# PotatoSpudowski/fastLLaMa

Measured on NVIDIA H100. Metric: tokens/sec LLaMA-7B q4_0 decode (n_batch=1, greedy), higher is better.
Workload: dtype u8

## Files before the change

fastllama_b200/csrc/fl_token_kernel.cu:

```cuda
#include <cuda_fp16.h>
#include <stdlib.h>

#include <algorithm>
#include <vector>

#include "fl_common.cuh"
#include "fl_decode.h"
#include "fl_decode_dev.cuh"
#include "fl_exact.cuh"
#include "fl_kernels.h"

#define TK_CW 16
#define TK_NT (TK_CW * 32)
#define TK_TG 4
#define TK_WPG 4
#define TK_GMAX 4
#define TK_CHB 32
#define TK_PW 4
#define TK_THREADS (TK_NT + 32 * TK_PW)
#define TK_REGS_CONSUMER 104
#define TK_REGS_PRODUCER 64

enum { TK_PH_MATVEC = 0, TK_PH_ATTN = 1 };

struct tk_phase {
    int kind;
    int nb, nchunks;
    uint32_t srow;
    int swiglu;
    int units[3];
    uint32_t row_bytes;
    fl_mv_args a;
    const float *q, *kcache, *vcache;
    float *out;
    int k_row_stride, n_head, head_dim, n_ctx;
    int head_split;
    int out_ll, out_seq, n_out_peer;
    float *out_peer[7];
    float scale;
};

struct tk_params {
    const tk_phase *phases;
    int n_phases;
    unsigned *grid_bar;
    unsigned *err;
    int rank, world;
    unsigned *ll_count;
    int n_ll;
    const uint16_t *exp_tab;
    unsigned long long *prof;
    unsigned *prof2;
    int S, Sg;
    uint32_t grid_magic, grid_shift, s_magic, s_shift;
    uint32_t slot_bytes;
    int diag;
    uint32_t off_y, off_red, off_rowbuf, off_cnt, off_sc, off_stage0;
};

__device__ __forceinline__ unsigned long long tk_now() {
    unsigned long long t;
    asm volatile("mov.u64 %0, %globaltimer;" : "=l"(t));
    return t;
}
__device__ __forceinline__ void tk_bar_consumers(int id) { asm volatile("bar.sync %0, %1;" ::"r"(id), "r"(TK_NT) : "memory"); }

__device__ __forceinline__ void tk_wait_ge(const unsigned *p, unsigned target, bool sys, unsigned *err, unsigned who) {
    unsigned long long t0 = 0;
    for (unsigned n = 1;; n++) {
        unsigned v;
        if (sys) asm volatile("ld.relaxed.sys.global.u32 %0, [%1];" : "=r"(v) : "l"(p) : "memory");
        else asm volatile("ld.acquire.gpu.global.u32 %0, [%1];" : "=r"(v) : "l"(p) : "memory");
        if ((int)(v - target) >= 0) return;
        if ((n & 1023u) == 0) {
            if (*(volatile unsigned *)err) return;
            const unsigned long long t = tk_now();
            if (t0 == 0) t0 = t;
            else if (t - t0 > 2000000000ull) {
                if (atomicExch(err, 1u) == 0u) { err[1] = who; err[2] = target; err[3] = v; err[4] = blockIdx.x; }
                return;
            }
        }
    }
}
__device__ __forceinline__ void tk_mbar_wait(uint32_t bar, uint32_t parity, unsigned *err, unsigned who, unsigned slot) {
    unsigned long long t0 = 0;
    for (unsigned n = 1; !fl_mbar_try_wait(bar, parity); n++) {
        if ((n & 4095u) == 0) {
            if (*(volatile unsigned *)err) return;
            const unsigned long long t = tk_now();
            if (t0 == 0) t0 = t;
            else if (t - t0 > 2000000000ull) {
                if (atomicExch(err, 1u) == 0u) { err[1] = who; err[2] = slot; err[3] = parity; err[4] = blockIdx.x; }
                return;
            }
        }
    }
}
__device__ __forceinline__ void tk_tag_wait(volatile uint32_t *tag, uint32_t want, unsigned *err, unsigned who, unsigned slot) {
    unsigned long long t0 = 0;
    for (unsigned n = 1; *tag != want; n++) {
        if ((n & 4095u) == 0) {
            if (*(volatile unsigned *)err) return;
            const unsigned long long t = tk_now();
            if (t0 == 0) t0 = t;
            else if (t - t0 > 2000000000ull) {
                if (atomicExch(err, 1u) == 0u) { err[1] = who; err[2] = slot; err[3] = want; err[4] = blockIdx.x; }
                return;
            }
        }
    }
}
__device__ __forceinline__ void tk_grid_sync(const tk_params &prm, unsigned target, unsigned) {
    tk_bar_consumers(13);
    if (threadIdx.x == 0) {
        asm volatile("red.release.gpu.global.add.u32 [%0], 1;" ::"l"(prm.grid_bar) : "memory");
        tk_wait_ge(prm.grid_bar, target, false, prm.err, 0x100u);
    }
    tk_bar_consumers(13);
}

struct tk_slice {
    int f0, f1, f2, n0, n1, n2, t0, t1, ntiles;
};
__device__ __forceinline__ uint32_t tk_div(uint32_t n, uint32_t magic, uint32_t shift) { return (magic ? __umulhi(n, magic) : n) >> shift; }
__device__ __forceinline__ tk_slice tk_make_slice_u(int m0, int m1, int m2, int lgG, uint32_t grid_magic, uint32_t grid_shift) {
    tk_slice sl;
    const unsigned U = (unsigned)(m0 + m1 + m2);
    const int u0 = (int)tk_div(U * blockIdx.x, grid_magic, grid_shift);
    const int u1 = (int)tk_div(U * (blockIdx.x + 1), grid_magic, grid_shift);
    const int rnd = (1 << lgG) - 1;
    fd_seg_span(u0, u1, 0, m0, sl.f0, sl.n0);
    fd_seg_span(u0, u1, m0, m1, sl.f1, sl.n1);
    fd_seg_span(u0, u1, m0 + m1, m2, sl.f2, sl.n2);
    sl.t0 = (sl.n0 + rnd) >> lgG;
    sl.t1 = sl.t0 + ((sl.n1 + rnd) >> lgG);
    sl.ntiles = sl.t1 + ((sl.n2 + rnd) >> lgG);
    return sl;
}
__device__ __forceinline__ void tk_tile_of(const tk_slice &sl, int G, int t, int &seg, int &unit0, int &nunits) {
    seg = (t < sl.t0) ? 0 : (t < sl.t1) ? 1 : 2;
    const int j = t - (seg == 0 ? 0 : seg == 1 ? sl.t0 : sl.t1);
    const int first = seg == 0 ? sl.f0 : seg == 1 ? sl.f1 : sl.f2;
    const int n = seg == 0 ? sl.n0 : seg == 1 ? sl.n1 : sl.n2;
    unit0 = first + j * G;
    nunits = min(G, n - j * G);
}

typedef fl_yx tk_yblock;

template <int E>
__device__ __forceinline__ void tk_load_vals(const float4 *p4, int u, float v[E], bool cg) {
#pragma unroll
    for (int k = 0; k < E / 4; k++) {
        const float4 t = cg ? __ldcg(p4 + (E / 4) * u + k) : __ldg(p4 + (E / 4) * u + k);
        v[4 * k + 0] = t.x; v[4 * k + 1] = t.y; v[4 * k + 2] = t.z; v[4 * k + 3] = t.w;
    }
}
template <int E>
__device__ __forceinline__ void tk_zero_vals(float v[E]) {
#pragma unroll
    for (int k = 0; k < E; k++) v[k] = 0.f;
}
template <int E>
__device__ __forceinline__ void tk_load_ll(const float *base, int u, float v[E], unsigned e, unsigned *err) {
    const uint4 *p = (const uint4 *)base + (size_t)(E / 2) * u;
    unsigned long long t0 = 0;
    for (unsigned n = 1;; n++) {
        uint4 t[E / 2];
#pragma unroll
        for (int k = 0; k < E / 2; k++)
            asm volatile("ld.relaxed.sys.global.v4.u32 {%0, %1, %2, %3}, [%4];" : "=r"(t[k].x), "=r"(t[k].y), "=r"(t[k].z), "=r"(t[k].w) : "l"(p + k) : "memory");
        bool ok = true;
#pragma unroll
        for (int k = 0; k < E / 2; k++) {
            ok = ok && t[k].y == e && t[k].w == e;
            v[2 * k] = __uint_as_float(t[k].x);
            v[2 * k + 1] = __uint_as_float(t[k].z);
        }
        if (ok) return;
        __nanosleep(n < 4 ? 40u : 200u);
        if ((n & 255u) == 0) {
            if (*(volatile unsigned *)err) return;
            const unsigned long long now = tk_now();
            if (t0 == 0) t0 = now;
            else if (now - t0 > 2000000000ull) {
                if (atomicExch(err, 1u) == 0u) { err[1] = 0x300u; err[2] = e; err[3] = t[0].y; err[4] = blockIdx.x; }
                return;
            }
        }
    }
}
template <int E>
__device__ __forceinline__ void tk_load_x(const fl_mv_args &A, int u, float v[E], unsigned ll_epoch, unsigned *err) {
    if (A.x_ll) tk_load_ll<E>(A.x, u, v, ll_epoch, err);
    else tk_load_vals<E>((const float4 *)A.x, u, v, true);
    if (A.xadd) {
        float w[E];
        tk_load_vals<E>((const float4 *)A.xadd, u, w, true);
#pragma unroll
        for (int k = 0; k < E; k++) v[k] = __fadd_rn(v[k], w[k]);
    }
}
template <int E>
__device__ __forceinline__ void tk_store_vals(float *dst, int u, const float v[E]) {
#pragma unroll
    for (int k = 0; k < E / 4; k++) ((float4 *)dst)[(E / 4) * u + k] = make_float4(v[4 * k], v[4 * k + 1], v[4 * k + 2], v[4 * k + 3]);
}
template <int E>
__device__ __forceinline__ void tk_quant(const float v[E], int u, bool valid, tk_yblock *ysm, int off) {
    float m0 = 0.f, m1 = 0.f;
#pragma unroll
    for (int k = 0; k < E; k += 2) { m0 = fmaxf(m0, fabsf(v[k])); m1 = fmaxf(m1, fabsf(v[k + 1])); }
    float amax = fmaxf(m0, m1);
    if (E <= 16) amax = fmaxf(amax, __shfl_xor_sync(0xffffffffu, amax, 1));
    if (E == 8) amax = fmaxf(amax, __shfl_xor_sync(0xffffffffu, amax, 2));
    const float d = __fdiv_rn(amax, 127.f);
    const float id = (amax != 0.0f) ? __fdiv_rn(127.f, amax) : 0.0f;
    int q[E], s0 = 0, s1 = 0;
#pragma unroll
    for (int k = 0; k < E; k += 2) {
        q[k] = max(-128, min(127, __float2int_rn(__fmul_rn(v[k], id))));
        q[k + 1] = max(-128, min(127, __float2int_rn(__fmul_rn(v[k + 1], id))));
        s0 += q[k]; s1 += q[k + 1];
    }
    int sum = s0 + s1;
    if (E <= 16) sum += __shfl_xor_sync(0xffffffffu, sum, 1);
    if (E == 8) sum += __shfl_xor_sync(0xffffffffu, sum, 2);
    if (valid) {
        constexpr int NW = E / 8;
        constexpr int UPB = 32 / E;
        tk_yblock *yb = ysm + u / UPB;
        const int part = u % UPB;
#pragma unroll
        for (int j = 0; j < NW; j++) {
            const uint32_t ya = (uint32_t)(q[8 * j + 0] & 0xFF) | ((uint32_t)(q[8 * j + 1] & 0xFF) << 8) | ((uint32_t)(q[8 * j + 2] & 0xFF) << 16) | ((uint32_t)(q[8 * j + 3] & 0xFF) << 24);
            const uint32_t yb4 = (uint32_t)(q[8 * j + 4] & 0xFF) | ((uint32_t)(q[8 * j + 5] & 0xFF) << 8) | ((uint32_t)(q[8 * j + 6] & 0xFF) << 16) | ((uint32_t)(q[8 * j + 7] & 0xFF) << 24);
            const int sa = q[8 * j + 0] + q[8 * j + 1] + q[8 * j + 2] + q[8 * j + 3], sb = q[8 * j + 4] + q[8 * j + 5] + q[8 * j + 6] + q[8 * j + 7];
            *(uint4 *)yb->q[NW * part + j] = make_uint4(ya, yb4, (uint32_t)(FX_MAGIC_I - off * sa), (uint32_t)(FX_MAGIC_I - off * sb));
        }
        if (part == 0) *(float2 *)&yb->d = make_float2(d, __fmul_rn(d, (float)sum));
    }
}
template <int E>
__device__ __forceinline__ void tk_prologue_nonorm(const fl_mv_args &A, int K, tk_yblock *ysm, int warp, int tid, unsigned lle, unsigned *err) {
    const int qoff = (A.type == FL_TYPE_Q4_0) ? 8 : 0;
    const int nu = K / E;
    if (E == 16 && A.pro != FL_PRO_SILUMUL && nu > TK_NT && nu <= 2 * TK_NT) {
        const int ua = tid, ub = tid + TK_NT;
        const bool vb = ub < nu, wb = TK_NT + warp * 32 < nu;
        float va[E], vv[E];
        tk_load_x<E>(A, ua, va, lle, err);
        if (vb) tk_load_x<E>(A, ub, vv, lle, err); else tk_zero_vals<E>(vv);
        if (A.sum_out && blockIdx.x == 0) { tk_store_vals<E>(A.sum_out, ua, va); if (vb) tk_store_vals<E>(A.sum_out, ub, vv); }
        tk_quant<E>(va, ua, true, ysm, qoff);
        if (wb) tk_quant<E>(vv, ub, vb, ysm, qoff);
        return;
    }
    for (int u0 = 0; u0 < nu; u0 += TK_NT) {
        if (u0 + warp * 32 >= nu) break;
        const int u = u0 + tid;
        const bool valid = u < nu;
        float v[E];
        if (valid) tk_load_x<E>(A, u, v, lle, err); else tk_zero_vals<E>(v);
        if (A.sum_out && blockIdx.x == 0 && valid) tk_store_vals<E>(A.sum_out, u, v);
        if (A.pro == FL_PRO_SILUMUL) {
            float bm[E];
            if (valid) tk_load_vals<E>((const float4 *)A.b, u, bm, true); else tk_zero_vals<E>(bm);
#pragma unroll
            for (int k = 0; k < E; k++) {
                const uint16_t hh = __half_as_ushort(__float2half_rn(v[k]));
                v[k] = __fmul_rn(__half2float(__ushort_as_half(__ldg(A.silu_tab + hh))), bm[k]);
            }
        }
        tk_quant<E>(v, u, valid, ysm, qoff);
    }
}

template <int RES>
__device__ __forceinline__ void tk_prologue_norm(const fl_mv_args &A, int K, tk_yblock *ysm, double *red, int warp, int lane, int tid, unsigned lle, unsigned *err) {
    const int qoff = (A.type == FL_TYPE_Q4_0) ? 8 : 0;
    constexpr int E = 8, NR = RES > 0 ? RES : 1;
    const int nu = K >> 3;
    float v[NR][E], gm[NR][E];
    double acc = 0.0;
    if (RES > 0) {
#pragma unroll
        for (int r = 0; r < NR; r++) {
            const int u = tid + r * TK_NT;
            if (u < nu) { tk_load_x<E>(A, u, v[r], lle, err); tk_load_vals<E>((const float4 *)A.gamma, u, gm[r], false); }
            else { tk_zero_vals<E>(v[r]); tk_zero_vals<E>(gm[r]); }
        }
#pragma unroll
        for (int r = 0; r < NR; r++)
#pragma unroll
            for (int k = 0; k < E; k++) acc += (double)__fmul_rn(v[r][k], v[r][k]);
    } else {
        for (int u = tid; u < nu; u += TK_NT) {
            tk_load_x<E>(A, u, v[0], lle, err);
#pragma unroll
            for (int k = 0; k < E; k++) acc += (double)__fmul_rn(v[0][k], v[0][k]);
        }
    }
    acc = fl_warp_sum_d(acc);
    if (lane == 0) red[warp] = acc;
    tk_bar_consumers(15);
    if (warp == 0) {
        double t = 0.0;
#pragma unroll
        for (int w = 0; w < TK_CW; w++) t += red[w];
        const float mean = (float)(t / (double)K);
        if (lane == 0) ((float *)(red + 16))[0] = __fdiv_rn(1.0f, __fsqrt_rn(__fadd_rn(mean, 1e-6f)));
    }
    tk_bar_consumers(15);
    const float scale = ((float *)(red + 16))[0];
    if (RES > 0) {
#pragma unroll
        for (int r = 0; r < NR; r++) {
            if (r * TK_NT + warp * 32 < nu) {
                const int u = tid + r * TK_NT;
                const bool valid = u < nu;
                if (A.sum_out && blockIdx.x == 0 && valid) tk_store_vals<E>(A.sum_out, u, v[r]);
#pragma unroll
                for (int k = 0; k < E; k++) v[r][k] = __fmul_rn(gm[r][k], __fmul_rn(v[r][k], scale));
                if (A.normed_out && blockIdx.x == 0 && valid) tk_store_vals<E>(A.normed_out, u, v[r]);
                tk_quant<E>(v[r], u, valid, ysm, qoff);
            }
        }
    } else {
        for (int u0 = 0; u0 < nu; u0 += TK_NT) {
            if (u0 + warp * 32 >= nu) break;
            const int u = u0 + tid;
            const bool valid = u < nu;
            if (valid) { tk_load_x<E>(A, u, v[0], lle, err); tk_load_vals<E>((const float4 *)A.gamma, u, gm[0], false); }
            else { tk_zero_vals<E>(v[0]); tk_zero_vals<E>(gm[0]); }
            if (A.sum_out && blockIdx.x == 0 && valid) tk_store_vals<E>(A.sum_out, u, v[0]);
#pragma unroll
            for (int k = 0; k < E; k++) v[0][k] = __fmul_rn(gm[0][k], __fmul_rn(v[0][k], scale));
            if (A.normed_out && blockIdx.x == 0 && valid) tk_store_vals<E>(A.normed_out, u, v[0]);
            tk_quant<E>(v[0], u, valid, ysm, qoff);
        }
    }
}

__device__ __forceinline__ void tk_prologue(const fl_mv_args &A, int K, tk_yblock *ysm, double *red, int warp, int lane, int tid, unsigned lle, unsigned *err) {
    const int nu8 = K >> 3;
    if (A.pro == FL_PRO_RMSNORM) {
        if (nu8 <= TK_NT) tk_prologue_norm<1>(A, K, ysm, red, warp, lane, tid, lle, err);
        else if (nu8 <= 2 * TK_NT) tk_prologue_norm<2>(A, K, ysm, red, warp, lane, tid, lle, err);
        else tk_prologue_norm<0>(A, K, ysm, red, warp, lane, tid, lle, err);
    } else if (nu8 <= TK_NT) {
        tk_prologue_nonorm<8>(A, K, ysm, warp, tid, lle, err);
    } else {
        tk_prologue_nonorm<16>(A, K, ysm, warp, tid, lle, err);
    }
}

__device__ __forceinline__ void tk_store_ll(float *slot, int row, float v, unsigned e, float *const *peers, int n_peers) {
    const unsigned uv = __float_as_uint(v);
    asm volatile("st.relaxed.sys.global.v2.u32 [%0], {%1, %2};" ::"l"(slot + 2 * row), "r"(uv), "r"(e) : "memory");
    for (int r = 0; r < n_peers; r++)
        asm volatile("st.relaxed.sys.global.v2.u32 [%0], {%1, %2};" ::"l"(peers[r] + 2 * row), "r"(uv), "r"(e) : "memory");
}
__device__ __forceinline__ float2 tk_epilogue_preload(const tk_phase &ph, int seg, int u, int n_past) {
    const fl_mv_args &A = ph.a;
    if (ph.swiglu) return make_float2(0.f, 0.f);
    const int r2 = 2 * u;
    if (A.epi == FL_EPI_QKV) {
        if (seg < 2) return __ldg((const float2 *)A.rope_cs + (size_t)n_past * (A.head_dim >> 1) + ((r2 % A.head_dim) >> 1));
        return make_float2(0.f, 0.f);
    }
    if (A.epi == FL_EPI_RESADD) {
        if (A.res_ll) {
            const float4 t = __ldcg((const float4 *)(A.res + 2 * r2));
            return make_float2(t.x, t.z);
        }
        return __ldcg((const float2 *)(A.res + r2));
    }
    return make_float2(0.f, 0.f);
}
__device__ __forceinline__ void tk_epilogue(const tk_phase &ph, int seg, int u, float a, float b, int n_past, float2 pre, unsigned ll_epoch) {
    const fl_mv_args &A = ph.a;
    if (ph.swiglu) {
        const uint16_t h = __half_as_ushort(__float2half_rn(a));
        const float o = __fmul_rn(__half2float(__ushort_as_half(__ldg(A.silu_tab + h))), b);
        if (A.out_ll) tk_store_ll(A.seg_dst[0], u, o, ll_epoch, A.dst_peer, A.n_dst_peer);
        else A.seg_dst[0][u] = o;
        return;
    }
    const int r2 = 2 * u;
    if (A.epi == FL_EPI_QKV) {
        if (seg < 2) {
            const float2 cs = pre;
            const float y0 = __fmaf_rn(a, cs.x, -__fmul_rn(b, cs.y));
            const float y1 = __fmaf_rn(a, cs.y, __fmul_rn(b, cs.x));
            float *o = (seg == 0) ? (A.seg_dst[0] + r2) : (A.kcache + (size_t)n_past * A.n_embd + r2);
            *(float2 *)o = make_float2(y0, y1);
        } else {
            A.vcache[(size_t)r2 * A.n_ctx + n_past] = a;
            A.vcache[(size_t)(r2 + 1) * A.n_ctx + n_past] = b;
        }
        return;
    }
    if (A.epi == FL_EPI_RESADD) {
        a = __fadd_rn(a, pre.x);
        b = __fadd_rn(b, pre.y);
    }
    if (A.out_ll) {
        tk_store_ll(A.seg_dst[seg], r2, a, ll_epoch, A.dst_peer, A.n_dst_peer);
        tk_store_ll(A.seg_dst[seg], r2 + 1, b, ll_epoch, A.dst_peer, A.n_dst_peer);
        return;
    }
    *(float2 *)(A.seg_dst[seg] + r2) = make_float2(a, b);
}

struct tk_stream {
    int first, n_g;
};
__device__ __forceinline__ tk_stream tk_stream_of(int g, int T0, int ntasks) {
    tk_stream st;
    st.first = ((g - (T0 & 3)) + 4) & 3;
    st.n_g = st.first < ntasks ? (ntasks - st.first + 3) >> 2 : 0;
    return st;
}
__device__ __forceinline__ void tk_slot_of(const tk_params &prm, int g, uint32_t idx, int &s, uint32_t &par) {
    const uint32_t q = tk_div(idx, prm.s_magic, prm.s_shift);
    s = (int)(idx - q * (uint32_t)prm.Sg) * TK_TG + g;
    par = q & 1u;
}

__device__ __forceinline__ unsigned tk_clock() {
    unsigned c;
    asm volatile("mov.u32 %0, %%clock;" : "=r"(c));
    return c;
}
template <int TYPE, bool PROF>
__device__ __forceinline__ void tk_consume(const tk_phase &ph, const tk_params &prm, const tk_slice &sl, int T0, uint32_t &cg, const tk_yblock *ysm,
                                           uint8_t *stage0, volatile uint32_t *tags, uint32_t bar0, int warp, int lane, unsigned *pw, unsigned lle) {
    unsigned c_begin = 0, c_wait = 0, c_dot = 0, c_tail = 0, c_rounds = 0, c_t = 0;
    if (PROF) { c_begin = tk_clock(); c_t = c_begin; }
    constexpr int BB = (TYPE == FL_TYPE_Q4_0) ? 20 : 24, QOFF = (TYPE == FL_TYPE_Q4_0) ? 4 : 8;
    const fl_mv_args &A = ph.a;
    const int S = prm.S;
    const int g = warp % TK_TG, wl = warp / TK_TG;
    const int r = lane >> 2, jj = lane & 3;
    const bool swiglu = ph.swiglu != 0;
    const int C = ph.nchunks, nb = ph.nb;
    const tk_stream st = tk_stream_of(g, T0, sl.ntiles);
    const int n_past = (A.epi == FL_EPI_QKV) ? *A.n_past : 0;
    const bool leader = swiglu ? ((lane & 3) == 0 && lane < 16) : ((lane & 7) == 0);
    const int pr = swiglu ? (lane >> 2) : (lane >> 3);
    const uint32_t row_off = (uint32_t)r * ph.srow + (uint32_t)(QOFF + 4 * jj);
    for (int k = wl; k < st.n_g; k += TK_WPG) {
        const int k0 = k - wl, n_r = min(TK_WPG, st.n_g - k0);
        int seg, unit0, nunits;
        tk_tile_of(sl, TK_GMAX, st.first + 4 * k, seg, unit0, nunits);
        float2 pre = make_float2(0.f, 0.f);
        if (leader && pr < nunits) pre = tk_epilogue_preload(ph, seg, unit0 + pr, n_past);
        float a0 = 0.0f, a1 = 0.0f, sm = 0.0f;
        for (int c = 0; c < C; c++) {
            int s;
            uint32_t par;
            const uint32_t idx = cg + (uint32_t)(k0 * C + c * n_r + wl);
            tk_slot_of(prm, g, idx, s, par);
            tk_tag_wait(tags + s, idx + 1u, prm.err, 0x600u + (unsigned)warp, (unsigned)s);
            tk_mbar_wait(bar0 + 8u * s, par, prm.err, 0x400u + (unsigned)warp, (unsigned)s);
            if (PROF) { const unsigned t = tk_clock(); c_wait += t - c_t; c_t = t; c_rounds++; }
            if (!(prm.diag & 2)) {
                const uint8_t *wp = stage0 + (size_t)s * prm.slot_bytes + row_off;
                const tk_yblock *yp = ysm + c * TK_CHB;
                const int nbc = min(TK_CHB, nb - c * TK_CHB);
#pragma unroll 8
                for (int i = 0; i < nbc; i++) {
                    const uint32_t w = *(const uint32_t *)(wp + i * BB);
                    const float dx = *(const float *)(wp + i * BB - (QOFF + 4 * jj));
                    const uint4 y = *(const uint4 *)yp[i].q[jj];
                    const float2 ds = *(const float2 *)&yp[i].d;
                    if (TYPE == FL_TYPE_Q4_1) sm = __fmaf_rn(*(const float *)(wp + i * BB - (QOFF + 4 * jj) + 4), ds.y, sm);
                    fx_block(w, __fmul_rn(dx, ds.x), y, a0, a1);
                }
            }
            __syncwarp();
            if (lane == 0) fl_mbar_arrive(bar0 + 8u * (S + s));
            if (PROF) { const unsigned t = tk_clock(); c_dot += t - c_t; c_t = t; }
        }
        float tot = fx_reduce(a0, a1);
        if (TYPE == FL_TYPE_Q4_1) tot = __fadd_rn(tot, sm);
        const float other = __shfl_down_sync(0xffffffffu, tot, swiglu ? 16 : 4);
        if (leader && pr < nunits) tk_epilogue(ph, seg, unit0 + pr, tot, other, n_past, pre, lle);
        if (PROF) { const unsigned t = tk_clock(); c_tail += t - c_t; c_t = t; }
    }
    cg += (uint32_t)(st.n_g * C);
    if (PROF && lane == 0 && pw) {
        pw[0] = 0; pw[1] = c_wait; pw[2] = c_dot; pw[3] = c_tail; pw[4] = c_rounds; pw[5] = tk_clock() - c_begin; pw[6] = (unsigned)sl.ntiles; pw[7] = 0;
    }
}

__device__ __forceinline__ void tk_attention(const tk_phase &ph, const tk_params &prm, float *sc, double *red, int head, int part_id, int warp, int lane, int tid, unsigned lle_out) {
    float *redf = (float *)(red + 20);
    const int hd = ph.head_dim;
    const int n_pos = *ph.a.n_past + 1;
    const float *q = ph.q + (size_t)head * hd;
    const float *kbase = ph.kcache + (size_t)head * hd;
    if (hd == 128) {
        float qe[4];
#pragma unroll
        for (int c = 0; c < 4; c++) qe[c] = __ldcg(q + lane + 32 * c);
        for (int j0 = warp * 8; j0 < n_pos; j0 += TK_CW * 8) {
            float kv[8][4], acc[8];
#pragma unroll
            for (int u = 0; u < 8; u++)
#pragma unroll
                for (int c = 0; c < 4; c++) kv[u][c] = __ldcg(kbase + (size_t)min(j0 + u, n_pos - 1) * ph.k_row_stride + lane + 32 * c);
#pragma unroll
            for (int u = 0; u < 8; u++) {
                acc[u] = 0.f;
#pragma unroll
                for (int c = 0; c < 4; c++) acc[u] = __fmaf_rn(kv[u][c], qe[c], acc[u]);
            }
#pragma unroll
            for (int u = 0; u < 8; u++) {
                const float a = fx_reduce_f32(acc[u]);
                if (lane == 0 && j0 + u < n_pos) sc[j0 + u] = __fmul_rn(a, ph.scale);
            }
        }
    } else {
        for (int j0 = warp * 4; j0 < n_pos; j0 += TK_CW * 4) {
            float acc[4] = {0.f, 0.f, 0.f, 0.f};
            for (int e = lane; e < hd; e += 32) {
                const float qe = __ldcg(q + e);
#pragma unroll
                for (int u = 0; u < 4; u++) acc[u] = __fmaf_rn(__ldcg(kbase + (size_t)min(j0 + u, n_pos - 1) * ph.k_row_stride + e), qe, acc[u]);
            }
#pragma unroll
            for (int u = 0; u < 4; u++) {
                const float a = fx_reduce_f32(acc[u]);
                if (lane == 0 && j0 + u < n_pos) sc[j0 + u] = __fmul_rn(a, ph.scale);
            }
        }
    }
    tk_bar_consumers(12);
    float mx = -INFINITY;
    for (int j = tid; j < n_pos; j += TK_NT) mx = fmaxf(mx, sc[j]);
    mx = fl_warp_max(mx);
    if (lane == 0) redf[warp] = mx;
    tk_bar_consumers(12);
    mx = redf[0];
    for (int w = 1; w < TK_CW; w++) mx = fmaxf(mx, redf[w]);
    double sum = 0.0;
    for (int j = tid; j < n_pos; j += TK_NT) {
        const uint16_t hh = __half_as_ushort(__float2half_rn(__fsub_rn(sc[j], mx)));
        const float e = __half2float(__ushort_as_half(__ldg(prm.exp_tab + hh)));
        sc[j] = e;
        sum += (double)e;
    }
    sum = fl_warp_sum_d(sum);
    if (lane == 0) red[warp] = sum;
    tk_bar_consumers(12);
    double tot = 0.0;
    for (int w = 0; w < TK_CW; w++) tot += red[w];
    const float inv = (float)(1.0 / tot);
    for (int j = tid; j < n_pos; j += TK_NT) sc[j] = __fmul_rn(sc[j], inv);
    tk_bar_consumers(12);
    const int dpc = hd / ph.head_split;
    const int np = n_pos & ~31, rem = n_pos - np, nma = fx_left_nma(rem);
    for (int dl = warp; dl < dpc; dl += TK_CW) {
        const int d = part_id * dpc + dl;
        const float *vrow = ph.vcache + ((size_t)head * hd + d) * ph.n_ctx;
        float acc = 0.0f;
        const float lx = (lane < rem) ? __ldcg(vrow + np + lane) : 0.0f, ly = (lane < rem) ? sc[np + lane] : 0.0f;
        const float lv = __fmul_rn(lx, ly);
        for (int k = lane; k < np; k += 32) acc = __fmaf_rn(__ldcg(vrow + k), sc[k], acc);
        float o = fx_reduce_f32(acc);
        for (int k = 0; k < nma; k++) o = __fadd_rn(o, __shfl_sync(0xffffffffu, lv, k));
        for (int k = nma; k < rem; k++) o = __fmaf_rn(__shfl_sync(0xffffffffu, lx, k), __shfl_sync(0xffffffffu, ly, k), o);
        if (lane == 0) {
            if (ph.out_ll) tk_store_ll(ph.out, head * hd + d, o, lle_out, ph.out_peer, ph.n_out_peer);
            else ph.out[(size_t)head * hd + d] = o;
        }
    }
}
__device__ __forceinline__ void tk_attention_prefetch(const tk_phase &ph, int head, int part_id, int tid) {
    const int hd = ph.head_dim, n_past = *ph.a.n_past;
    const int kl = (hd * 4 + 127) / 128;
    for (int i = tid; i < n_past * kl; i += TK_NT) {
        const float *p = ph.kcache + (size_t)(i / kl) * ph.k_row_stride + (size_t)head * hd + (i % kl) * 32;
        asm volatile("prefetch.global.L2 [%0];" ::"l"(p));
    }
    const int dpc = hd / ph.head_split;
    const int vl = (n_past * 4 + 127) / 128;
    for (int i = tid; i < dpc * vl; i += TK_NT) {
        const float *p = ph.vcache + ((size_t)head * hd + part_id * dpc + i / vl) * ph.n_ctx + (i % vl) * 32;
        asm volatile("prefetch.global.L2 [%0];" ::"l"(p));
    }
}

template <bool PROF>
__global__ void __launch_bounds__(TK_THREADS, 1) k_decode_token(const tk_params prm) {
    extern __shared__ __align__(128) uint8_t smem[];
    uint64_t *bars = (uint64_t *)smem;
    volatile uint32_t *tags = (volatile uint32_t *)(smem + (size_t)16 * prm.S);
    tk_yblock *ysm = (tk_yblock *)(smem + prm.off_y);
    double *red = (double *)(smem + prm.off_red);
    float *sc = (float *)(smem + prm.off_sc);
    uint8_t *stage0 = smem + prm.off_stage0;
    __shared__ __align__(16) tk_phase phs[2];
    __shared__ tk_slice sl_sh;
    const int S = prm.S;
    const int warp = threadIdx.x >> 5, lane = threadIdx.x & 31;
    const uint32_t bar0 = fl_smem_u32(bars);

    if (warp >= TK_CW) {
        asm volatile("setmaxnreg.dec.sync.aligned.u32 %0;" ::"n"(TK_REGS_PRODUCER));
        const int pg = warp - TK_CW;
        if (pg == 0 && lane == 0) {
            for (int s = 0; s < S; s++) {
                fl_mbar_init(bar0 + 8u * s, 1);
                fl_mbar_init(bar0 + 8u * (S + s), 1);
                tags[s] = 0u;
            }
            fl_mbar_fence_init();
        }
        __syncwarp();
        asm volatile("bar.sync 14, %0;" ::"r"(TK_THREADS) : "memory");
        {
            const uint64_t pol = fl_policy_evict_first();
            int T0 = 0;
            uint32_t cg = 0;
            for (int pi = 0; pi < prm.n_phases; pi++) {
                const tk_phase *gp = prm.phases + pi;
                if (__ldg(&gp->kind) != TK_PH_MATVEC) continue;
                const int swiglu = __ldg(&gp->swiglu), C = __ldg(&gp->nchunks), nb = __ldg(&gp->nb), type = __ldg(&gp->a.type);
                const int m0 = __ldg(&gp->units[0]), m1 = __ldg(&gp->units[1]), m2 = __ldg(&gp->units[2]);
                const uint32_t row_bytes = __ldg(&gp->row_bytes), srow = __ldg(&gp->srow);
                const uint32_t bb = (type == FL_TYPE_Q4_0) ? 20u : 24u;
                const uint8_t *w0 = (const uint8_t *)__ldg((const unsigned long long *)&gp->a.seg_w[0]);
                const uint8_t *w1 = (const uint8_t *)__ldg((const unsigned long long *)&gp->a.seg_w[1]);
                const uint8_t *w2 = (const uint8_t *)__ldg((const unsigned long long *)&gp->a.seg_w[2]);
                const tk_slice sl = tk_make_slice_u(m0, m1, m2, 2, prm.grid_magic, prm.grid_shift);
                const tk_stream st = tk_stream_of(pg, T0, sl.ntiles);
                for (int k0 = 0; k0 < st.n_g; k0 += TK_WPG) {
                    const int n_r = min(TK_WPG, st.n_g - k0);
                    for (int c = 0; c < C; c++) {
                        const uint32_t cbytes = (uint32_t)min(TK_CHB, nb - c * TK_CHB) * bb;
                        for (int wl = 0; wl < n_r; wl++) {
                            int seg, unit0, nunits;
                            tk_tile_of(sl, TK_GMAX, st.first + 4 * (k0 + wl), seg, unit0, nunits);
                            int s;
                            uint32_t par;
                            const uint32_t idx = cg + (uint32_t)(k0 * C + c * n_r + wl);
                            tk_slot_of(prm, pg, idx, s, par);
                            const uint8_t *src = nullptr;
                            if (lane < 8) {
                                if (swiglu) { if ((lane & 3) < nunits) src = ((lane < 4) ? w0 : w1) + (size_t)(unit0 + (lane & 3)) * row_bytes; }
                                else if (lane < 2 * nunits) src = (seg == 0 ? w0 : seg == 1 ? w1 : w2) + (size_t)(2 * unit0 + lane) * row_bytes;
                            }
                            if (lane == 0) {
                                tk_mbar_wait(bar0 + 8u * (S + s), par ^ 1u, prm.err, 0x500u + (unsigned)pg, (unsigned)s);
                                tags[s] = idx + 1u;
                                if (prm.diag & 1) fl_mbar_arrive(bar0 + 8u * s);
                                else fl_mbar_expect_tx(bar0 + 8u * s, 2u * (uint32_t)nunits * cbytes);
                            }
                            __syncwarp();
                            if (src && !(prm.diag & 1))
                                fl_bulk_g2s_hint(fl_smem_u32(stage0 + (size_t)s * prm.slot_bytes + (size_t)lane * srow), src + (size_t)c * (TK_CHB * bb), cbytes, bar0 + 8u * s, pol);
                        }
                    }
                }
                cg += (uint32_t)(st.n_g * C);
                T0 += sl.ntiles;
            }
        }
        return;
    }

    asm volatile("setmaxnreg.inc.sync.aligned.u32 %0;" ::"n"(TK_REGS_CONSUMER));
    const int tid = threadIdx.x;
    static_assert(sizeof(tk_phase) % 4 == 0 && sizeof(tk_phase) / 4 <= TK_NT, "descriptor copy is one word per thread");
    if (warp == TK_CW - 1)
        for (int i = lane; i < (int)(sizeof(tk_phase) / 4); i += 32) ((uint32_t *)&phs[0])[i] = ((const uint32_t *)&prm.phases[0])[i];
    tk_bar_consumers(15);
    asm volatile("bar.sync 14, %0;" ::"r"(TK_THREADS) : "memory");
    int T0 = 0;
    uint32_t cg = 0;
    unsigned epoch = 0;
    unsigned ll_base = 0;
    if (prm.n_ll > 0) asm volatile("ld.relaxed.gpu.global.u32 %0, [%1];" : "=r"(ll_base) : "l"(prm.ll_count) : "memory");
    unsigned *err = prm.err;
    for (int pi = 0; pi < prm.n_phases; pi++) {
        const tk_phase &ph = phs[pi & 1];
        unsigned long long *pr = (prm.prof && tid == 0) ? prm.prof + ((size_t)pi * gridDim.x + blockIdx.x) * 4 : nullptr;
        if (pr) pr[0] = tk_now();
        const bool attn_here = ph.kind == TK_PH_ATTN && (int)blockIdx.x < ph.n_head * ph.head_split;
        const int a_head = attn_here ? (int)blockIdx.x / ph.head_split : 0, a_part = attn_here ? (int)blockIdx.x % ph.head_split : 0;
        if (attn_here) tk_attention_prefetch(ph, a_head, a_part, tid);
        const bool ll_in = ph.kind == TK_PH_MATVEC && ph.a.x_ll;
        const unsigned lle_in = ll_in ? ll_base + (unsigned)ph.a.x_seq + 1u : 0u;
        const unsigned lle_out = ph.kind == TK_PH_MATVEC ? (ph.a.out_ll ? ll_base + (unsigned)ph.a.out_seq + 1u : 0u) : (ph.out_ll ? ll_base + (unsigned)ph.out_seq + 1u : 0u);
        if (pi > 0 && ll_in) {
            tk_bar_consumers(13);
        } else if (pi > 0) {
            epoch++;
            if (!(prm.diag & 4)) tk_grid_sync(prm, epoch * gridDim.x, 0u);
            else tk_bar_consumers(13);
        }
        if (pr) pr[1] = tk_now();
        uint32_t next_word = 0;
        const bool copies = tid < (int)(sizeof(tk_phase) / 4) && pi + 1 < prm.n_phases;
        if (copies) next_word = __ldcg((const uint32_t *)&prm.phases[pi + 1] + tid);
        if (ph.kind == TK_PH_ATTN) {
            if (attn_here && !(prm.diag & 16)) tk_attention(ph, prm, sc, red, a_head, a_part, warp, lane, tid, lle_out);
            if (copies) ((uint32_t *)&phs[(pi + 1) & 1])[tid] = next_word;
            tk_bar_consumers(15);
            if (pr) pr[2] = pr[3] = tk_now();
            continue;
        }
        const int K = ph.nb * 32;
        if (tid == TK_NT - 1) sl_sh = tk_make_slice_u(ph.units[0], ph.units[1], ph.units[2], 2, prm.grid_magic, prm.grid_shift);
        if (!(prm.diag & 8)) tk_prologue(ph.a, K, ysm, red, warp, lane, tid, lle_in, err);
        if (copies) ((uint32_t *)&phs[(pi + 1) & 1])[tid] = next_word;
        tk_bar_consumers(15);
        if (pr) pr[2] = tk_now();
        const tk_slice &sl = sl_sh;
        unsigned *pw = (PROF && prm.prof2) ? prm.prof2 + (((size_t)pi * gridDim.x + blockIdx.x) * TK_CW + warp) * 8 : nullptr;
        if (ph.a.type == FL_TYPE_Q4_0) tk_consume<FL_TYPE_Q4_0, PROF>(ph, prm, sl, T0, cg, ysm, stage0, tags, bar0, warp, lane, pw, lle_out);
        else                           tk_consume<FL_TYPE_Q4_1, PROF>(ph, prm, sl, T0, cg, ysm, stage0, tags, bar0, warp, lane, pw, lle_out);
        T0 += sl.ntiles;
        if (pr) pr[3] = tk_now();
    }
    if (prm.n_ll > 0 && blockIdx.x == 0 && tid == 0) *prm.ll_count = ll_base + (unsigned)prm.n_ll;
}

struct fl_token_plan_impl {
    tk_phase *d_phases = nullptr;
    unsigned *d_bar = nullptr;
    unsigned *h_err = nullptr;
    unsigned long long *d_prof = nullptr;
    unsigned *d_prof2 = nullptr;
    tk_params prm;
    size_t smem = 0;
    int n_kernels = 0;
};

static void tk_magic(uint32_t d, uint32_t &magic, uint32_t &shift) {
    uint32_t k = 0;
    while ((2u << k) <= d) k++;
    shift = k;
    magic = ((d & (d - 1)) == 0) ? 0u : (uint32_t)((((uint64_t)1 << (32 + k)) + d - 1) / d);
}

static int tk_geometry(tk_phase &ph, size_t &tile_bytes) {
    const fl_mv_args &a = ph.a;
    const int bb = fl_block_bytes(a.type);
    const int nb = a.K / 32;
    const size_t row_bytes = a.row_stride_bytes ? a.row_stride_bytes : (size_t)nb * bb;
    FL_REQUIRE(bb > 0 && a.K > 0 && a.K % 32 == 0 && row_bytes % 16 == 0, "token kernel: unsupported matrix K=%d", a.K);
    const uint32_t chunk_bytes = (uint32_t)std::min(nb, TK_CHB) * bb;
    FL_REQUIRE(chunk_bytes % 16 == 0 && ((size_t)nb * bb) % 16 == 0, "token kernel: K=%d gives row pieces that are not multiples of 16 bytes", a.K);
    const uint32_t srow = (chunk_bytes / 16) % 2 ? chunk_bytes : chunk_bytes + 16;
    ph.units[0] = ph.units[1] = ph.units[2] = 0;
    if (ph.swiglu) {
        ph.units[0] = a.seg_rows[0];
    } else {
        for (int i = 0; i < a.nseg; i++) {
            FL_REQUIRE(a.seg_rows[i] > 0 && a.seg_rows[i] % 2 == 0, "token kernel: segment %d has an odd row count", i);
            ph.units[i] = a.seg_rows[i] / 2;
        }
    }
    for (int i = 0; i < a.nseg; i++) {
        FL_REQUIRE(((uintptr_t)a.seg_w[i] & 15) == 0, "token kernel: segment %d is not 16-byte aligned", i);
        FL_REQUIRE(a.epi == FL_EPI_QKV || ph.swiglu || ((uintptr_t)a.seg_dst[i] & 7) == 0, "token kernel: output %d is not 8-byte aligned", i);
    }
    FL_REQUIRE(a.epi != FL_EPI_RESADD || ((uintptr_t)a.res & 7) == 0, "token kernel: residual is not 8-byte aligned");
    FL_REQUIRE((long)ph.units[0] + ph.units[1] + ph.units[2] < (1 << 23), "token kernel: too many rows");
    ph.kind = TK_PH_MATVEC;
    ph.nb = nb; ph.nchunks = (nb + TK_CHB - 1) / TK_CHB; ph.srow = srow; ph.row_bytes = (uint32_t)row_bytes;
    tile_bytes = (size_t)2 * TK_GMAX * srow;
    return 0;
}

int flk_token_plan_create(const fl_token_step *steps, int n_steps, const uint16_t *silu_tab, const uint16_t *exp_tab, const void *rope_cs, unsigned *epoch_counter, void **out) {
    std::vector<tk_phase> phases((size_t)n_steps);
    for (int i = 0; i < n_steps; i++) {
        tk_phase &ph = phases[i];
        memset(&ph, 0, sizeof(ph));
        if (steps[i].kind == 1) {
            ph.kind = TK_PH_ATTN;
            ph.q = steps[i].q; ph.kcache = steps[i].kcache; ph.vcache = steps[i].vcache; ph.out = steps[i].out;
            ph.k_row_stride = steps[i].k_row_stride; ph.n_head = steps[i].n_head; ph.head_dim = steps[i].head_dim; ph.n_ctx = steps[i].n_ctx;
            ph.scale = steps[i].scale;
            ph.a.n_past = steps[i].n_past;
            ph.out_ll = steps[i].out_ll; ph.out_seq = steps[i].out_seq; ph.n_out_peer = steps[i].n_out_peer;
            for (int r = 0; r < 7; r++) ph.out_peer[r] = steps[i].out_peer[r];
        } else {
            ph.kind = TK_PH_MATVEC;
            ph.a = steps[i].mv;
            ph.a.silu_tab = silu_tab;
            ph.a.rope_cs = rope_cs;
        }
    }
    for (int i = 0; i < n_steps; i++)
        if (phases[i].kind == TK_PH_MATVEC && phases[i].a.swiglu) {
            const fl_mv_args &a = phases[i].a;
            FL_REQUIRE(a.nseg == 2 && a.epi == FL_EPI_STORE && a.seg_rows[0] == a.seg_rows[1], "token kernel: a swiglu step needs two equal segments and a plain store");
            phases[i].swiglu = 1;
        }
    for (int i = 0; i + 1 < n_steps; i++) {
        tk_phase &p0 = phases[i], &p1 = phases[i + 1];
        if (p0.kind != TK_PH_MATVEC || p1.kind != TK_PH_MATVEC || p0.swiglu) continue;
        const fl_mv_args &a = p0.a;
        if (a.nseg == 2 && a.epi == FL_EPI_STORE && a.seg_rows[0] == a.seg_rows[1] && p1.a.pro == FL_PRO_SILUMUL && p1.a.x == a.seg_dst[0] &&
            p1.a.b == a.seg_dst[1] && p1.a.K == a.seg_rows[0] && p1.a.xadd == nullptr) {
            p0.swiglu = 1;
            p1.a.pro = FL_PRO_PLAIN;
            p1.a.b = nullptr;
        }
    }
    size_t max_tile = 0, max_y = 0;
    int max_ctx = 0;
    int sm_count = 0;
    {
        int dev0 = 0;
        FL_CUDA_OK(cudaGetDevice(&dev0));
        FL_CUDA_OK(cudaDeviceGetAttribute(&sm_count, cudaDevAttrMultiProcessorCount, dev0));
    }
    for (int i = 0; i < n_steps; i++) {
        tk_phase &ph = phases[i];
        if (ph.kind == TK_PH_ATTN) {
            FL_REQUIRE(ph.n_ctx % 4 == 0 && ph.head_dim >= 32 && ph.head_dim <= 256 && (ph.head_dim & (ph.head_dim - 1)) == 0 && ph.n_head <= sm_count,
                       "token kernel: unsupported attention shape");
            ph.head_split = 1;
            for (int c = 4; c > 1; c /= 2)
                if (c * ph.n_head <= sm_count && ph.head_dim / c >= 32) { ph.head_split = c; break; }
            max_ctx = std::max(max_ctx, ph.n_ctx);
        } else {
            size_t tb = 0;
            if (tk_geometry(ph, tb)) return -1;
            max_tile = std::max(max_tile, tb);
            max_y = std::max(max_y, (size_t)ph.nb * sizeof(tk_yblock));
        }
    }
    int dev = 0, sm = 0, optin = 0;
    FL_CUDA_OK(cudaGetDevice(&dev));
    FL_CUDA_OK(cudaDeviceGetAttribute(&sm, cudaDevAttrMultiProcessorCount, dev));
    FL_CUDA_OK(cudaDeviceGetAttribute(&optin, cudaDevAttrMaxSharedMemoryPerBlockOptin, dev));
    fl_token_plan_impl *pl = new fl_token_plan_impl();
    struct plan_guard {
        fl_token_plan_impl *p;
        ~plan_guard() { if (p) flk_token_plan_destroy(p); }
    } guard{pl};
    tk_params &p = pl->prm;
    const size_t slot = (max_tile + 127) & ~(size_t)127;
    int S = 64;
    if (getenv("FASTLLAMA_B200_TK_SLOTS")) S = std::max(8, std::min(64, atoi(getenv("FASTLLAMA_B200_TK_SLOTS")) / 4 * 4));
    size_t off = 0;
    for (;; S -= 4) {
        if (S < 8) { fl_set_error("token kernel: tiles of %zu bytes do not fit shared memory", slot); return -1; }
        p.off_y = ((size_t)(2 * S) * 8 + (size_t)S * 4 + 127) & ~(size_t)127;
        p.off_red = (p.off_y + max_y + 127) & ~(size_t)127;
        p.off_sc = (p.off_red + 32 * sizeof(double) + 127) & ~(size_t)127;
        off = (p.off_sc + ((size_t)max_ctx + 32) * sizeof(float) + 127) & ~(size_t)127;
        if (off + (size_t)S * slot <= (size_t)optin - 1024) break;
    }
    p.off_rowbuf = p.off_cnt = 0;
    p.off_stage0 = (uint32_t)off;
    p.S = S;
    p.Sg = S / TK_TG;
    tk_magic((uint32_t)sm, p.grid_magic, p.grid_shift);
    tk_magic((uint32_t)p.Sg, p.s_magic, p.s_shift);
    p.slot_bytes = (uint32_t)slot;
    p.n_phases = n_steps;
    p.exp_tab = exp_tab;
    p.diag = getenv("FASTLLAMA_B200_TK_DIAG") ? atoi(getenv("FASTLLAMA_B200_TK_DIAG")) : 0;
    pl->smem = off + (size_t)S * slot;
    FL_CUDA_OK(cudaMalloc((void **)&pl->d_phases, sizeof(tk_phase) * (size_t)n_steps));
    FL_CUDA_OK(cudaMemcpy(pl->d_phases, phases.data(), sizeof(tk_phase) * (size_t)n_steps, cudaMemcpyHostToDevice));
    FL_CUDA_OK(cudaMalloc((void **)&pl->d_bar, 256));
    p.phases = pl->d_phases;
    p.grid_bar = pl->d_bar;
    FL_CUDA_OK(cudaMemset(pl->d_bar, 0, 256));
    FL_CUDA_OK(cudaHostAlloc((void **)&pl->h_err, 64, cudaHostAllocMapped));
    memset(pl->h_err, 0, 64);
    FL_CUDA_OK(cudaHostGetDevicePointer((void **)&p.err, pl->h_err, 0));
    p.rank = 0; p.world = 1; p.ll_count = epoch_counter; p.n_ll = 0;
    for (int i = 0; i < n_steps; i++) {
        const tk_phase &ph = phases[i];
        if (ph.kind == TK_PH_MATVEC) {
            if (ph.a.out_ll) p.n_ll = std::max(p.n_ll, ph.a.out_seq + 1);
            if (ph.a.x_ll) p.n_ll = std::max(p.n_ll, ph.a.x_seq + 1);
            if (ph.a.out_ll && ph.a.nseg != 1 && !ph.swiglu) { fl_set_error("token kernel: an LL output needs a single segment (or a w1|w3 pair)"); return -1; }
        } else if (ph.out_ll) p.n_ll = std::max(p.n_ll, ph.out_seq + 1);
    }
    if (p.n_ll > 0 && !epoch_counter) { fl_set_error("token kernel: steps use LL vectors but no epoch counter was given (fl_token_plan_create_ll)"); return -1; }
    p.prof = nullptr;
    p.prof2 = nullptr;
    if (getenv("FASTLLAMA_B200_TOKEN_PROF")) {
        FL_CUDA_OK(cudaMalloc((void **)&pl->d_prof, sizeof(unsigned long long) * 4 * (size_t)n_steps * sm));
        FL_CUDA_OK(cudaMemset(pl->d_prof, 0, sizeof(unsigned long long) * 4 * (size_t)n_steps * sm));
        p.prof = pl->d_prof;
        const size_t n2 = (size_t)n_steps * sm * TK_CW * 8;
        FL_CUDA_OK(cudaMalloc((void **)&pl->d_prof2, n2 * sizeof(unsigned)));
        FL_CUDA_OK(cudaMemset(pl->d_prof2, 0, n2 * sizeof(unsigned)));
        p.prof2 = pl->d_prof2;
    }
    cudaFuncAttributes fa;
    FL_CUDA_OK(cudaFuncGetAttributes(&fa, k_decode_token<false>));
    FL_CUDA_OK(cudaFuncSetAttribute(k_decode_token<false>, cudaFuncAttributeMaxDynamicSharedMemorySize, optin - (int)fa.sharedSizeBytes));
    FL_CUDA_OK(cudaFuncGetAttributes(&fa, k_decode_token<true>));
    FL_CUDA_OK(cudaFuncSetAttribute(k_decode_token<true>, cudaFuncAttributeMaxDynamicSharedMemorySize, optin - (int)fa.sharedSizeBytes));
    FL_REQUIRE((size_t)TK_REGS_CONSUMER * TK_NT + (size_t)TK_REGS_PRODUCER * 32 * TK_PW <= (size_t)fa.numRegs * TK_THREADS,
               "token kernel: register re-allocation (%d x %d + %d x %d) exceeds the launch allocation (%d x %d)", TK_REGS_CONSUMER, TK_NT, TK_REGS_PRODUCER,
               32 * TK_PW, fa.numRegs, TK_THREADS);
    int per_sm = 0;
    FL_CUDA_OK(cudaOccupancyMaxActiveBlocksPerMultiprocessor(&per_sm, k_decode_token<false>, TK_THREADS, pl->smem));
    if (per_sm < 1) { const size_t need = pl->smem; fl_set_error("token kernel: one CTA per SM does not fit (smem %zu)", need); return -1; }
    pl->n_kernels = sm;
    guard.p = nullptr;
    *out = pl;
    return 0;
}

int flk_token_plan_launch(cudaStream_t st, void *plan) {
    fl_token_plan_impl *pl = (fl_token_plan_impl *)plan;
    FL_CUDA_OK(cudaMemsetAsync(pl->d_bar, 0, 4, st));
    void *args[] = {(void *)&pl->prm};
    const void *fn = pl->prm.prof2 ? (const void *)k_decode_token<true> : (const void *)k_decode_token<false>;
    FL_CUDA_OK(cudaLaunchCooperativeKernel(fn, dim3(pl->n_kernels), dim3(TK_THREADS), args, pl->smem, st));
    fl_count_launch();
    return 0;
}

int flk_token_plan_profile(void *plan, unsigned long long *out, size_t max_words, int *n_ctas) {
    fl_token_plan_impl *pl = (fl_token_plan_impl *)plan;
    FL_REQUIRE(pl && pl->d_prof, "token plan was created without FASTLLAMA_B200_TOKEN_PROF");
    const size_t words = (size_t)4 * pl->prm.n_phases * pl->n_kernels;
    FL_REQUIRE(max_words >= words, "profile buffer too small (%zu words needed)", words);
    FL_CUDA_OK(cudaMemcpy(out, pl->d_prof, words * sizeof(unsigned long long), cudaMemcpyDeviceToHost));
    *n_ctas = pl->n_kernels;
    return 0;
}

int flk_token_plan_profile2(void *plan, unsigned *out, size_t max_words) {
    fl_token_plan_impl *pl = (fl_token_plan_impl *)plan;
    FL_REQUIRE(pl && pl->d_prof2, "token plan was created without FASTLLAMA_B200_TOKEN_PROF");
    const size_t words = (size_t)pl->prm.n_phases * pl->n_kernels * TK_CW * 8;
    FL_REQUIRE(max_words >= words, "profile buffer too small (%zu words needed)", words);
    FL_CUDA_OK(cudaMemcpy(out, pl->d_prof2, words * sizeof(unsigned), cudaMemcpyDeviceToHost));
    return 0;
}

int flk_token_plan_error(void *plan) {
    fl_token_plan_impl *pl = (fl_token_plan_impl *)plan;
    if (!pl || !pl->h_err) return 0;
    const volatile unsigned *e = pl->h_err;
    if (e[0])
        fl_set_error("token kernel timeout: %s (code 0x%x), waited for / slot %u, last saw / parity %u, CTA %u, rank %d of %d",
                     (e[1] & 0x700u) == 0x600u ? "consumer warp waiting for a slot tag" : (e[1] & 0x700u) == 0x400u ? "consumer warp waiting for a weight tile" : (e[1] & 0x700u) == 0x500u ? "producer waiting for a free ring slot" :
                     (e[1] & 0x300u) == 0x300u ? "LL vector element" : "grid barrier counter", e[1], e[2], e[3], e[4], pl->prm.rank, pl->prm.world);
    return (int)e[0];
}

int flk_token_plan_destroy(void *plan) {
    fl_token_plan_impl *pl = (fl_token_plan_impl *)plan;
    if (!pl) return 0;
    if (pl->d_phases) cudaFree(pl->d_phases);
    if (pl->d_bar) cudaFree(pl->d_bar);
    if (pl->h_err) cudaFreeHost(pl->h_err);
    if (pl->d_prof) cudaFree(pl->d_prof);
    if (pl->d_prof2) cudaFree(pl->d_prof2);
    delete pl;
    return 0;
}
```

Measured before the change: 403.0.

## Replace grid barrier before attention with per-head group barriers via head-aligned QKV split

When a fused QKV matvec directly feeds attention, the matvec rows are assigned so each CTA produces Q/K/V rows for a single head slice (hgu units per CTA). The attention phase then waits only on a per-head counter reached by the head_split CTAs that produced that head, instead of a full grid barrier. This aims to cut grid-wide synchronization latency in decode. The trade-off is that the fixed head-aligned partition can leave some CTAs idle or unbalanced, it needs more barrier memory, and each launch now resets a larger barrier buffer.

```diff
diff --git a/fastllama_b200/csrc/fl_token_kernel.cu b/fastllama_b200/csrc/fl_token_kernel.cu
--- a/fastllama_b200/csrc/fl_token_kernel.cu
+++ b/fastllama_b200/csrc/fl_token_kernel.cu
@@ -29,12 +29,14 @@
     uint32_t srow;
     int swiglu;
     int units[3];
+    int hgu;
     uint32_t row_bytes;
     fl_mv_args a;
     const float *q, *kcache, *vcache;
     float *out;
     int k_row_stride, n_head, head_dim, n_ctx;
     int head_split;
+    int group_bar;
     int out_ll, out_seq, n_out_peer;
     float *out_peer[7];
     float scale;
@@ -119,20 +121,35 @@
     }
     tk_bar_consumers(13);
 }
+__device__ __forceinline__ void tk_group_sync(const tk_params &prm, int head, unsigned target) {
+    tk_bar_consumers(13);
+    if (threadIdx.x == 0) {
+        unsigned *cnt = prm.grid_bar + 32 * (1 + head);
+        asm volatile("red.release.gpu.global.add.u32 [%0], 1;" ::"l"(cnt) : "memory");
+        tk_wait_ge(cnt, target, false, prm.err, 0x200u);
+    }
+    tk_bar_consumers(13);
+}
 
 struct tk_slice {
     int f0, f1, f2, n0, n1, n2, t0, t1, ntiles;
 };
 __device__ __forceinline__ uint32_t tk_div(uint32_t n, uint32_t magic, uint32_t shift) { return (magic ? __umulhi(n, magic) : n) >> shift; }
-__device__ __forceinline__ tk_slice tk_make_slice_u(int m0, int m1, int m2, int lgG, uint32_t grid_magic, uint32_t grid_shift) {
+__device__ __forceinline__ tk_slice tk_make_slice_u(int m0, int m1, int m2, int hgu, int lgG, uint32_t grid_magic, uint32_t grid_shift) {
     tk_slice sl;
-    const unsigned U = (unsigned)(m0 + m1 + m2);
-    const int u0 = (int)tk_div(U * blockIdx.x, grid_magic, grid_shift);
-    const int u1 = (int)tk_div(U * (blockIdx.x + 1), grid_magic, grid_shift);
     const int rnd = (1 << lgG) - 1;
-    fd_seg_span(u0, u1, 0, m0, sl.f0, sl.n0);
-    fd_seg_span(u0, u1, m0, m1, sl.f1, sl.n1);
-    fd_seg_span(u0, u1, m0 + m1, m2, sl.f2, sl.n2);
+    if (hgu > 0) {
+        const int f = (int)blockIdx.x * hgu, n = f + hgu <= m0 ? hgu : 0;
+        sl.f0 = sl.f1 = sl.f2 = f;
+        sl.n0 = sl.n1 = sl.n2 = n;
+    } else {
+        const unsigned U = (unsigned)(m0 + m1 + m2);
+        const int u0 = (int)tk_div(U * blockIdx.x, grid_magic, grid_shift);
+        const int u1 = (int)tk_div(U * (blockIdx.x + 1), grid_magic, grid_shift);
+        fd_seg_span(u0, u1, 0, m0, sl.f0, sl.n0);
+        fd_seg_span(u0, u1, m0, m1, sl.f1, sl.n1);
+        fd_seg_span(u0, u1, m0 + m1, m2, sl.f2, sl.n2);
+    }
     sl.t0 = (sl.n0 + rnd) >> lgG;
     sl.t1 = sl.t0 + ((sl.n1 + rnd) >> lgG);
     sl.ntiles = sl.t1 + ((sl.n2 + rnd) >> lgG);
@@ -631,13 +648,13 @@
                 const tk_phase *gp = prm.phases + pi;
                 if (__ldg(&gp->kind) != TK_PH_MATVEC) continue;
                 const int swiglu = __ldg(&gp->swiglu), C = __ldg(&gp->nchunks), nb = __ldg(&gp->nb), type = __ldg(&gp->a.type);
-                const int m0 = __ldg(&gp->units[0]), m1 = __ldg(&gp->units[1]), m2 = __ldg(&gp->units[2]);
+                const int m0 = __ldg(&gp->units[0]), m1 = __ldg(&gp->units[1]), m2 = __ldg(&gp->units[2]), hgu = __ldg(&gp->hgu);
                 const uint32_t row_bytes = __ldg(&gp->row_bytes), srow = __ldg(&gp->srow);
                 const uint32_t bb = (type == FL_TYPE_Q4_0) ? 20u : 24u;
                 const uint8_t *w0 = (const uint8_t *)__ldg((const unsigned long long *)&gp->a.seg_w[0]);
                 const uint8_t *w1 = (const uint8_t *)__ldg((const unsigned long long *)&gp->a.seg_w[1]);
                 const uint8_t *w2 = (const uint8_t *)__ldg((const unsigned long long *)&gp->a.seg_w[2]);
-                const tk_slice sl = tk_make_slice_u(m0, m1, m2, 2, prm.grid_magic, prm.grid_shift);
+                const tk_slice sl = tk_make_slice_u(m0, m1, m2, hgu, 2, prm.grid_magic, prm.grid_shift);
                 const tk_stream st = tk_stream_of(pg, T0, sl.ntiles);
                 for (int k0 = 0; k0 < st.n_g; k0 += TK_WPG) {
                     const int n_r = min(TK_WPG, st.n_g - k0);
@@ -683,7 +700,7 @@
     asm volatile("bar.sync 14, %0;" ::"r"(TK_THREADS) : "memory");
     int T0 = 0;
     uint32_t cg = 0;
-    unsigned epoch = 0;
+    unsigned epoch = 0, gepoch = 0;
     unsigned ll_base = 0;
     if (prm.n_ll > 0) asm volatile("ld.relaxed.gpu.global.u32 %0, [%1];" : "=r"(ll_base) : "l"(prm.ll_count) : "memory");
     unsigned *err = prm.err;
@@ -699,6 +716,10 @@
         const unsigned lle_out = ph.kind == TK_PH_MATVEC ? (ph.a.out_ll ? ll_base + (unsigned)ph.a.out_seq + 1u : 0u) : (ph.out_ll ? ll_base + (unsigned)ph.out_seq + 1u : 0u);
         if (pi > 0 && ll_in) {
             tk_bar_consumers(13);
+        } else if (pi > 0 && ph.kind == TK_PH_ATTN && ph.group_bar) {
+            gepoch++;
+            if (attn_here && !(prm.diag & 4)) tk_group_sync(prm, a_head, gepoch * (unsigned)ph.head_split);
+            else tk_bar_consumers(13);
         } else if (pi > 0) {
             epoch++;
             if (!(prm.diag & 4)) tk_grid_sync(prm, epoch * gridDim.x, 0u);
@@ -716,7 +737,7 @@
             continue;
         }
         const int K = ph.nb * 32;
-        if (tid == TK_NT - 1) sl_sh = tk_make_slice_u(ph.units[0], ph.units[1], ph.units[2], 2, prm.grid_magic, prm.grid_shift);
+        if (tid == TK_NT - 1) sl_sh = tk_make_slice_u(ph.units[0], ph.units[1], ph.units[2], ph.hgu, 2, prm.grid_magic, prm.grid_shift);
         if (!(prm.diag & 8)) tk_prologue(ph.a, K, ysm, red, warp, lane, tid, lle_in, err);
         if (copies) ((uint32_t *)&phs[(pi + 1) & 1])[tid] = next_word;
         tk_bar_consumers(15);
@@ -734,6 +755,7 @@
 struct fl_token_plan_impl {
     tk_phase *d_phases = nullptr;
     unsigned *d_bar = nullptr;
+    size_t bar_bytes = 0;
     unsigned *h_err = nullptr;
     unsigned long long *d_prof = nullptr;
     unsigned *d_prof2 = nullptr;
@@ -817,7 +839,7 @@
         }
     }
     size_t max_tile = 0, max_y = 0;
-    int max_ctx = 0;
+    int max_ctx = 0, max_heads = 0;
     int sm_count = 0;
     {
         int dev0 = 0;
@@ -833,11 +855,24 @@
             for (int c = 4; c > 1; c /= 2)
                 if (c * ph.n_head <= sm_count && ph.head_dim / c >= 32) { ph.head_split = c; break; }
             max_ctx = std::max(max_ctx, ph.n_ctx);
+            max_heads = std::max(max_heads, ph.n_head);
         } else {
             size_t tb = 0;
             if (tk_geometry(ph, tb)) return -1;
             max_tile = std::max(max_tile, tb);
             max_y = std::max(max_y, (size_t)ph.nb * sizeof(tk_yblock));
+        }
+    }
+    for (int i = 0; i + 1 < n_steps; i++) {
+        tk_phase &p0 = phases[i], &p1 = phases[i + 1];
+        if (p0.kind != TK_PH_MATVEC || p1.kind != TK_PH_ATTN) continue;
+        const fl_mv_args &a = p0.a;
+        const int hd = p1.head_dim, split = p1.head_split, n = p1.n_head * hd;
+        if (a.epi == FL_EPI_QKV && a.nseg == 3 && !a.x_ll && !a.out_ll && !p1.out_ll && a.head_dim == hd && a.n_embd == n && a.n_ctx == p1.n_ctx &&
+            a.seg_rows[0] == n && a.seg_rows[1] == n && a.seg_rows[2] == n && p1.q == a.seg_dst[0] && p1.kcache == a.kcache && p1.vcache == a.vcache &&
+            p1.k_row_stride == n && (hd / split) % 2 == 0 && 8 * p1.n_head * split >= 7 * sm_count) {
+            p0.hgu = hd / split / 2;
+            p1.group_bar = 1;
         }
     }
     int dev = 0, sm = 0, optin = 0;
@@ -875,10 +910,11 @@
     pl->smem = off + (size_t)S * slot;
     FL_CUDA_OK(cudaMalloc((void **)&pl->d_phases, sizeof(tk_phase) * (size_t)n_steps));
     FL_CUDA_OK(cudaMemcpy(pl->d_phases, phases.data(), sizeof(tk_phase) * (size_t)n_steps, cudaMemcpyHostToDevice));
-    FL_CUDA_OK(cudaMalloc((void **)&pl->d_bar, 256));
+    pl->bar_bytes = (size_t)128 * (1 + max_heads);
+    FL_CUDA_OK(cudaMalloc((void **)&pl->d_bar, pl->bar_bytes));
     p.phases = pl->d_phases;
     p.grid_bar = pl->d_bar;
-    FL_CUDA_OK(cudaMemset(pl->d_bar, 0, 256));
+    FL_CUDA_OK(cudaMemset(pl->d_bar, 0, pl->bar_bytes));
     FL_CUDA_OK(cudaHostAlloc((void **)&pl->h_err, 64, cudaHostAllocMapped));
     memset(pl->h_err, 0, 64);
     FL_CUDA_OK(cudaHostGetDevicePointer((void **)&p.err, pl->h_err, 0));
@@ -922,7 +958,7 @@
 
 int flk_token_plan_launch(cudaStream_t st, void *plan) {
     fl_token_plan_impl *pl = (fl_token_plan_impl *)plan;
-    FL_CUDA_OK(cudaMemsetAsync(pl->d_bar, 0, 4, st));
+    FL_CUDA_OK(cudaMemsetAsync(pl->d_bar, 0, pl->bar_bytes, st));
     void *args[] = {(void *)&pl->prm};
     const void *fn = pl->prm.prof2 ? (const void *)k_decode_token<true> : (const void *)k_decode_token<false>;
     FL_CUDA_OK(cudaLaunchCooperativeKernel(fn, dim3(pl->n_kernels), dim3(TK_THREADS), args, pl->smem, st));
@@ -956,6 +992,7 @@
     if (e[0])
         fl_set_error("token kernel timeout: %s (code 0x%x), waited for / slot %u, last saw / parity %u, CTA %u, rank %d of %d",
                      (e[1] & 0x700u) == 0x600u ? "consumer warp waiting for a slot tag" : (e[1] & 0x700u) == 0x400u ? "consumer warp waiting for a weight tile" : (e[1] & 0x700u) == 0x500u ? "producer waiting for a free ring slot" :
+                     (e[1] & 0x700u) == 0x200u ? "head-group barrier counter" :
                      (e[1] & 0x300u) == 0x300u ? "LL vector element" : "grid barrier counter", e[1], e[2], e[3], e[4], pl->prm.rank, pl->prm.world);
     return (int)e[0];
 }
```

Result: faster. 407.5 (median of 6 runs) (+1.1%).
